# chathurawidanage/harp

Measured on AMD Instinct MI355X. Metric: sec/iteration K-means (N=1e8, d=100, K=1e4), lower is better.
Workload: dtype bf16; 1 GPU; model=kmeans-allreduce, N=100000000, d=100, K=10000, global_batch=100000000, parallelism=dp1

## Files before the change

### csrc/kmeans.hip

```cpp
#include "common.h"

#include <type_traits>

namespace {

constexpr float KM_BIG = 1.0e38f;
constexpr int KM_ONES = 4;

__device__ __forceinline__ float keyed(float v, unsigned idx) {
  return __uint_as_float((__float_as_uint(v) & ~0xFu) | idx);
}

template <int KS, int G, int WAVES_, int RG>
struct KMCfg {
  static constexpr int DP = KS * 16;
  static constexpr int CPR = KS * 2;
  static constexpr int TILE = RG * 32;
  static constexpr int WAVES = WAVES_;
  static constexpr int THREADS = WAVES_ * 64;
  static constexpr int TILE_BYTES = TILE * DP * 2;
  static constexpr int DMA_INSTR = TILE * CPR / 64;
  static constexpr int PTS = WAVES_ * G * 32;
  static_assert((TILE * CPR) % 64 == 0, "tile must be whole 1-KiB DMA pieces");
};

template <class C>
__device__ __forceinline__ void stage_dma(const __bf16* __restrict__ cm2, int tile, char* lds, int wave, int lane) {
#pragma unroll
  for (int j0 = 0; j0 < C::DMA_INSTR; j0 += C::WAVES) {
    const int j = j0 + wave;
    if (C::DMA_INSTR % C::WAVES == 0 || j < C::DMA_INSTR) {
      const int q = j * 64 + lane;
      const int row = q / C::CPR;
      int c = q - row * C::CPR - ((row >> 3) & 1);
      if (c < 0) c += C::CPR;
      const __bf16* src = cm2 + ((size_t)tile * C::TILE + row) * C::DP + c * 8;
      __builtin_amdgcn_global_load_lds((const void __attribute__((address_space(1)))*)src,
                                       (void __attribute__((address_space(3)))*)(lds + j * 1024), 16, 0, 0);
    }
  }
}

template <int KS, int G, int WAVES, int RG, int PIPE, int PRIO = 0>
__global__ __launch_bounds__(WAVES * 64) void kmeans_assign_kernel(
    const __bf16* __restrict__ X, long ldx, const __bf16* __restrict__ Cm2, long N, int ntiles, int tail_rg,
    int dcount, int* __restrict__ labels, float* __restrict__ sums, int ld_sums, float* __restrict__ obj_partial,
    float* __restrict__ mind) {
  using C = KMCfg<KS, G, WAVES, RG>;
  __shared__ __attribute__((aligned(16))) char smem[2 * C::TILE_BYTES + WAVES * 4];
  const int tid = threadIdx.x, lane = tid & 63, wave = tid >> 6;
  const int r = lane & 31, h = lane >> 5;
  const int srot = (r >> 3) & 1;
  const long pbase = ((long)blockIdx.x * WAVES + wave) * (G * 32);

  if constexpr (PRIO)
    if (__builtin_amdgcn_readfirstlane(tid) >= WAVES * 32) __builtin_amdgcn_s_setprio(1);
  stage_dma<C>(Cm2, 0, smem, wave, lane);

  bf16x8 xf[G][KS];
#pragma unroll
  for (int g = 0; g < G; ++g) {
    long p = pbase + g * 32 + r;
    if (p > N - 1) p = N - 1;
    const bf16x8* row = (const bf16x8*)(X + p * ldx);
#pragma unroll
    for (int s = 0; s < KS; ++s) xf[g][s] = row[2 * s + h];
  }

  float best[G];
  int bestt[G];
#pragma unroll
  for (int g = 0; g < G; ++g) { best[g] = KM_BIG; bestt[g] = 0; }
  auto tile_argmin = [&](const floatx16& ac, int g, int tg) {
    float m = keyed(ac[0], 0u);
#pragma unroll
    for (int q = 1; q < 16; ++q) m = fminf(m, keyed(ac[q], (unsigned)q));
    if (m < best[g]) { best[g] = m; bestt[g] = tg; }
  };

  int aoff[KS];
#pragma unroll
  for (int s = 0; s < KS; ++s) {
    int cp = 2 * s + h + srot;
    if (cp >= C::CPR) cp -= C::CPR;
    aoff[s] = (r * C::CPR + cp) * 16;
  }

  asm volatile("s_waitcnt vmcnt(0)" ::: "memory");
  __syncthreads();

  const int nfull = tail_rg ? ntiles - 1 : ntiles;
  for (int t = 0; t < nfull; ++t) {
    if (t + 1 < ntiles) stage_dma<C>(Cm2, t + 1, smem + ((t + 1) & 1) * C::TILE_BYTES, wave, lane);
    const char* buf = smem + (t & 1) * C::TILE_BYTES;
    bf16x8 af[2][KS];
#pragma unroll
    for (int s = 0; s < KS; ++s) af[0][s] = *(const bf16x8*)(buf + aoff[s]);
    if constexpr (PIPE > 0) {
      constexpr int NI = RG * G;
      floatx16 acc[2];
#pragma unroll
      for (int q = 0; q < 16; ++q) acc[0][q] = 0.f;
#pragma unroll
      for (int s = 0; s < KS; ++s) acc[0] = __builtin_amdgcn_mfma_f32_32x32x16_bf16(af[0][s], xf[0][s], acc[0], 0, 0, 0);
#pragma unroll
      for (int i = 0; i < NI; ++i) {
        const int rg = i / G, g = i % G;
        if (g == 0 && rg + 1 < RG) {
          const char* nb = buf + (rg + 1) * 32 * C::CPR * 16;
#pragma unroll
          for (int s = 0; s < KS; ++s) af[(rg + 1) & 1][s] = *(const bf16x8*)(nb + aoff[s]);
        }
        if (i + 1 < NI) {
          const int rg1 = (i + 1) / G, g1 = (i + 1) % G;
          floatx16& an = acc[(i + 1) & 1];
#pragma unroll
          for (int q = 0; q < 16; ++q) an[q] = 0.f;
#pragma unroll
          for (int s = 0; s < KS; ++s) an = __builtin_amdgcn_mfma_f32_32x32x16_bf16(af[rg1 & 1][s], xf[g1][s], an, 0, 0, 0);
        }
        tile_argmin(acc[i & 1], g, t * RG + rg);
        if constexpr (PIPE == 2) {
#pragma unroll
          for (int s = 0; s < KS; ++s) {
            __builtin_amdgcn_sched_group_barrier(0x008, 1, 0);
            __builtin_amdgcn_sched_group_barrier(0x002, 4, 0);
          }
        }
      }
    } else
#pragma unroll
    for (int rg = 0; rg < RG; ++rg) {
      if (rg + 1 < RG) {
        const char* nb = buf + (rg + 1) * 32 * C::CPR * 16;
#pragma unroll
        for (int s = 0; s < KS; ++s) af[(rg + 1) & 1][s] = *(const bf16x8*)(nb + aoff[s]);
      }
      const int tg = t * RG + rg;
#pragma unroll
      for (int g = 0; g < G; ++g) {
        floatx16 acc = {0.f, 0.f, 0.f, 0.f, 0.f, 0.f, 0.f, 0.f, 0.f, 0.f, 0.f, 0.f, 0.f, 0.f, 0.f, 0.f};
#pragma unroll
        for (int s = 0; s < KS; ++s)
          acc = __builtin_amdgcn_mfma_f32_32x32x16_bf16(af[rg & 1][s], xf[g][s], acc, 0, 0, 0);
        tile_argmin(acc, g, tg);
      }
    }
    asm volatile("s_waitcnt vmcnt(0)" ::: "memory");
    __syncthreads();
  }
  if (tail_rg) {
    const int t = ntiles - 1;
    const char* buf = smem + (t & 1) * C::TILE_BYTES;
    for (int rg = 0; rg < tail_rg; ++rg) {
      const char* nb = buf + rg * 32 * C::CPR * 16;
      bf16x8 af[KS];
#pragma unroll
      for (int s = 0; s < KS; ++s) af[s] = *(const bf16x8*)(nb + aoff[s]);
      const int tg = t * RG + rg;
#pragma unroll
      for (int g = 0; g < G; ++g) {
        floatx16 acc = {0.f, 0.f, 0.f, 0.f, 0.f, 0.f, 0.f, 0.f, 0.f, 0.f, 0.f, 0.f, 0.f, 0.f, 0.f, 0.f};
#pragma unroll
        for (int s = 0; s < KS; ++s) acc = __builtin_amdgcn_mfma_f32_32x32x16_bf16(af[s], xf[g][s], acc, 0, 0, 0);
        tile_argmin(acc, g, tg);
      }
    }
  }

  int lab[G];
  float local_obj = 0.f;
#pragma unroll
  for (int g = 0; g < G; ++g) {
    float xs = 0.f;
#pragma unroll
    for (int s = 0; s < KS; ++s)
#pragma unroll
      for (int j = 0; j < 8; ++j) {
        const float v = (float)xf[g][s][j];
        xs = fmaf(v, v, xs);
      }
    xs += __shfl_xor(xs, 32, 64);
    xs -= (float)KM_ONES;
    const float ob = __shfl_xor(best[g], 32, 64);
    const int obt = __shfl_xor(bestt[g], 32, 64);
    const bool take = h ? (ob <= best[g]) : (ob < best[g]);
    const float bv = take ? ob : best[g];
    const int bt = take ? obt : bestt[g];
    const int hw = take ? (1 - h) : h;
    const unsigned reg = __float_as_uint(bv) & 0xFu;
    const int idx = bt * 32 + (int)(reg & 3u) + 8 * (int)(reg >> 2) + 4 * hw;
    lab[g] = idx;
    const long p = pbase + g * 32 + r;
    if (h == 0 && p < N) {
      labels[p] = idx;
      local_obj += fmaxf(bv + xs, 0.f);
      if (mind) mind[p] = bv + xs;
    }
  }
  if (obj_partial) {
    local_obj = wave_sum(local_obj);
    float* red = (float*)(smem + 2 * C::TILE_BYTES);
    if (lane == 0) red[wave] = local_obj;
    __syncthreads();
    if (tid == 0) {
      float acc = 0.f;
#pragma unroll
      for (int w = 0; w < WAVES; ++w) acc += red[w];
      obj_partial[blockIdx.x] = acc;
    }
  }

  if (sums) {
#pragma unroll
    for (int g = 0; g < G; ++g) {
      for (int i = 0; i < 32; ++i) {
        const long p = pbase + g * 32 + i;
        if (p >= N) break;
        const int l = __shfl(lab[g], i, 64);
        const __bf16* xr = X + p * ldx;
        float* sr = sums + (long)l * ld_sums;
        for (int c = lane; c <= dcount; c += 64) atomicAdd(sr + c, (float)xr[c]);
      }
    }
  }
}

__global__ void kmeans_normalize_kernel(const float* __restrict__ sums, int ld, float* __restrict__ c,
                                        int Kr, int d, float* __restrict__ counts) {
  const int row = blockIdx.x * (blockDim.x >> 6) + (threadIdx.x >> 6);
  const int lane = threadIdx.x & 63;
  if (row >= Kr) return;
  const float cnt = sums[(long)row * ld + d];
  if (counts && lane == 0) counts[row] = cnt;
  if (cnt > 0.f) {
    const float inv = 1.0f / cnt;
    for (int j = lane; j < d; j += 64) c[(long)row * d + j] = sums[(long)row * ld + j] * inv;
  }
}

__global__ void kmeans_prepare_kernel(const float* __restrict__ c, int K, int d, int Kp, int dp,
                                      __bf16* __restrict__ Cm2, float* __restrict__ cn) {
  const int row = blockIdx.x * (blockDim.x >> 6) + (threadIdx.x >> 6);
  const int lane = threadIdx.x & 63;
  if (row >= Kp) return;
  float s = 0.f;
  for (int j = lane; j < d; j += 64) {
    float v = row < K ? c[(long)row * d + j] : 0.f;
    const float bf = (float)(__bf16)v;
    s = fmaf(bf, bf, s);
    Cm2[(long)row * dp + j] = (__bf16)(-2.0f * bf);
  }
  s = wave_sum(s);
  if (row >= K) s = KM_BIG;
  const __bf16 hi = (__bf16)s;
  const float r1 = s - (float)hi;
  const __bf16 mid = (__bf16)r1;
  const __bf16 lo = (__bf16)(r1 - (float)mid);
  for (int j = d + lane; j < dp; j += 64) {
    __bf16 v = (__bf16)0.f;
    if (j == d + 1) v = hi;
    else if (j == d + 2) v = mid;
    else if (j == d + 3) v = lo;
    Cm2[(long)row * dp + j] = v;
  }
  if (lane == 0) cn[row] = s;
}

__device__ __forceinline__ unsigned long long splitmix64(unsigned long long z) {
  z += 0x9E3779B97F4A7C15ull;
  z = (z ^ (z >> 30)) * 0xBF58476D1CE4E5B9ull;
  z = (z ^ (z >> 27)) * 0x94D049BB133111EBull;
  return z ^ (z >> 31);
}

__global__ void uniform_rows_bf16_kernel(__bf16* __restrict__ X, long N, int d, int dp, float lo,
                                         float hi, unsigned long long seed, long row0, int one_col) {
  const long total = N * (long)dp;
  for (long i = blockIdx.x * (long)blockDim.x + threadIdx.x; i < total; i += (long)gridDim.x * blockDim.x) {
    const long row = i / dp;
    const int col = (int)(i - row * dp);
    float v = 0.f;
    if (col < d) {
      const unsigned long long z = splitmix64(seed ^ ((unsigned long long)(row0 + row) * 0x100000001B3ull + col));
      v = lo + (hi - lo) * (float)((z >> 40) * (1.0 / 16777216.0));
    } else if (one_col && col < d + KM_ONES) {
      v = 1.0f;
    }
    X[i] = (__bf16)v;
  }
}

constexpr int KW_CB = 256, KW_RG = KW_CB / 32;

template <int G, int DC>
struct KWCfg {
  static constexpr int KS = DC / 16;
  static constexpr int CPR = DC / 8;
  static constexpr int TILE_BYTES = KW_CB * DC * 2;
  static constexpr int DMA = KW_CB * CPR / 64;
  static constexpr int PTS = 4 * G * 32;
};

template <int CPR>
__device__ __forceinline__ int wide_rot(int row) {
  return CPR == 4 ? (row >> 2) & 3 : CPR == 8 ? (row >> 1) & 7 : CPR == 16 ? row & 15 : (row >> 3) & 1;
}

template <class C>
__device__ __forceinline__ void stage_dma_wide(const __bf16* __restrict__ cm2, int dp, int row0, int kp, int f,
                                               char* lds, int wave, int lane) {
#pragma unroll
  for (int j0 = 0; j0 < C::DMA; j0 += 4) {
    const int j = j0 + wave;
    const int q = j * 64 + lane;
    const int row = q / C::CPR;
    int c = q - row * C::CPR - wide_rot<C::CPR>(row);
    if (c < 0) c += C::CPR;
    int gr = row0 + row;
    if (gr > kp - 1) gr = kp - 1;
    const __bf16* src = cm2 + (size_t)gr * dp + f * (C::CPR * 8) + c * 8;
    __builtin_amdgcn_global_load_lds((const void __attribute__((address_space(1)))*)src,
                                     (void __attribute__((address_space(3)))*)(lds + j * 1024), 16, 0, 0);
  }
}

template <int G, int DC, int OCC>
__global__ __launch_bounds__(256, OCC) void kmeans_assign_wide_kernel(
    const __bf16* __restrict__ X, long ldx, const __bf16* __restrict__ Cm2, long N, int dp, int kswept, int kp,
    int nkb, unsigned long long* __restrict__ keys) {
  using C = KWCfg<G, DC>;
  constexpr int KS = C::KS;
  __shared__ __attribute__((aligned(16))) char smem[2 * C::TILE_BYTES];
  const int tid = threadIdx.x, lane = tid & 63, wave = tid >> 6;
  const int r = lane & 31, h = lane >> 5;
  const int srot = (r >> 3) & 1;
  const long id = blockIdx.x;
  const long xcd = id & 7, round = id >> 3;
  const long pb = (round / nkb) * 8 + xcd;
  const int kb = (int)(round % nkb);
  const long npb = (N + C::PTS - 1) / C::PTS;
  if (pb >= npb) return;
  const int row0 = kb * KW_CB;
  const int live_rg = (kswept - row0) >= KW_CB ? KW_RG : (kswept - row0 + 31) / 32;
  const long pbase = pb * C::PTS + wave * (G * 32);
  const int nst = dp / DC;

  stage_dma_wide<C>(Cm2, dp, row0, kp, 0, smem, wave, lane);
  const bf16x8* xrow[G];
#pragma unroll
  for (int g = 0; g < G; ++g) {
    long p = pbase + g * 32 + r;
    if (p > N - 1) p = N - 1;
    xrow[g] = (const bf16x8*)(X + p * ldx);
  }
  bf16x8 xf[2][G][KS];
#pragma unroll
  for (int g = 0; g < G; ++g)
#pragma unroll
    for (int k = 0; k < KS; ++k) xf[0][g][k] = xrow[g][2 * k + h];
  floatx16 acc[KW_RG][G];
#pragma unroll
  for (int a = 0; a < KW_RG; ++a)
#pragma unroll
    for (int g = 0; g < G; ++g)
#pragma unroll
// ... 285 lines not shown
                                       (void __attribute__((address_space(3)))*)(xb + j * 1024), 16, 0, 0);
    }
  };
  floatx16 acc[RGW][G];
#pragma unroll
  for (int a = 0; a < RGW; ++a)
#pragma unroll
    for (int g = 0; g < G; ++g)
#pragma unroll
      for (int q = 0; q < 16; ++q) acc[a][g][q] = 0.f;
  int aoff[KS];
#pragma unroll
  for (int k = 0; k < KS; ++k) aoff[k] = (r * CPR + (2 * k + h + wide_rot<CPR>(r)) % CPR) * 16;
#pragma unroll
  for (int q = 0; q < NBUF - 1; ++q)
    if (q < nst) issue(q, q);
  float xs[G];
#pragma unroll
  for (int g = 0; g < G; ++g) xs[g] = 0.f;
  for (int f = 0; f < nst; ++f) {
    const int younger = (nst - 1 - f) < (NBUF - 2) ? (nst - 1 - f) : (NBUF - 2);
    if (younger >= 2) asm volatile("s_waitcnt vmcnt(%0)" ::"n"(2 * OPS) : "memory");
    else if (younger == 1) asm volatile("s_waitcnt vmcnt(%0)" ::"n"(OPS) : "memory");
    else asm volatile("s_waitcnt vmcnt(0)" ::: "memory");
    __syncthreads();
    if (f + NBUF - 1 < nst) issue(f + NBUF - 1, (f + NBUF - 1) % NBUF);
    const char* buf = smem + (f % NBUF) * SBYTES;
    const char* xb = buf + C::TILE_BYTES + pwo * CPR * 16;
    const char* cb = buf + rgo * 32 * CPR * 16;
    bf16x8 xf[G][KS];
#pragma unroll
    for (int g = 0; g < G; ++g)
#pragma unroll
      for (int k = 0; k < KS; ++k) xf[g][k] = *(const bf16x8*)(xb + g * 32 * CPR * 16 + aoff[k]);
#pragma unroll
    for (int g = 0; g < G; ++g)
#pragma unroll
      for (int k = 0; k < KS; ++k)
#pragma unroll
        for (int j = 0; j < 8; ++j) xs[g] = fmaf((float)xf[g][k][j], (float)xf[g][k][j], xs[g]);
    bf16x8 af[2][KS];
#pragma unroll
    for (int k = 0; k < KS; ++k) af[0][k] = *(const bf16x8*)(cb + aoff[k]);
#pragma unroll
    for (int rg = 0; rg < RGW; ++rg) {
      if (rg + 1 < RGW) {
        const char* nb = cb + (rg + 1) * 32 * CPR * 16;
#pragma unroll
        for (int k = 0; k < KS; ++k) af[(rg + 1) & 1][k] = *(const bf16x8*)(nb + aoff[k]);
      }
      if (rg < live_rg) {
#pragma unroll
        for (int g = 0; g < G; ++g)
#pragma unroll
          for (int k = 0; k < KS; ++k)
            acc[rg][g] = __builtin_amdgcn_mfma_f32_32x32x16_bf16(af[rg & 1][k], xf[g][k], acc[rg][g], 0, 0, 0);
      }
    }
  }
  float xsg[G];
#pragma unroll
  for (int g = 0; g < G; ++g) xsg[g] = xs[g] + __shfl_xor(xs[g], 32, 64) - (float)KM_ONES;
#pragma unroll
  for (int g = 0; g < G; ++g) {
    float best = KM_BIG;
    int bestt = 0;
#pragma unroll
    for (int rg = 0; rg < RGW; ++rg) {
      if (rg >= live_rg) break;
      float m = keyed(acc[rg][g][0], 0u);
#pragma unroll
      for (int q = 1; q < 16; ++q) m = fminf(m, keyed(acc[rg][g][q], (unsigned)q));
      if (m < best) {
        best = m;
        bestt = rg;
      }
    }
    const float ob = __shfl_xor(best, 32, 64);
    const int obt = __shfl_xor(bestt, 32, 64);
    const bool take = h ? (ob <= best) : (ob < best);
    const float bv = take ? ob : best;
    const int bt = take ? obt : bestt;
    const int hw = take ? (1 - h) : h;
    const unsigned reg = __float_as_uint(bv) & 0xFu;
    const int idx = row0 + (rgo + bt) * 32 + (int)(reg & 3u) + 8 * (int)(reg >> 2) + 4 * hw;
    const long p = pbase + g * 32 + r;
    if (h == 0 && p < N && live_rg > 0) {
      const float dist = fmaxf(bv + xsg[g], 0.f);
      const unsigned long long key = ((unsigned long long)__float_as_uint(dist) << 32) | (unsigned)idx;
      __hip_atomic_fetch_min(keys + p, key, __ATOMIC_RELAXED, __HIP_MEMORY_SCOPE_AGENT);
    }
  }
}

template <int G, int DC, int NBUF>
int launch_wide8(const void* X, long ldx, const void* Cm2, long N, int dp, int kswept, int kp,
                 unsigned long long* keys, hipStream_t s) {
  constexpr int XROWS = 4 * G * 32;
  if (dp % DC || (ldx * 2) % 16) return HARP_EBADARG;
  const long npb = (N + XROWS - 1) / XROWS;
  const int nkb = (kswept + KW_CB - 1) / KW_CB;
  const long rounds = (npb + 7) / 8 * nkb;
  kmeans_assign_wide8_kernel<G, DC, NBUF><<<dim3((unsigned)(rounds * 8)), dim3(512), 0, s>>>(
      (const __bf16*)X, ldx, (const __bf16*)Cm2, N, dp, kswept, kp, nkb, keys);
  return harp_launch_status();
}

template <int G, int DC, int NBUF>
int launch_wide_lds(const void* X, long ldx, const void* Cm2, long N, int dp, int kswept, int kp,
                    unsigned long long* keys, hipStream_t s) {
  constexpr int XROWS = 4 * G * 32;
  constexpr int SBYTES = KW_CB * DC * 2 + XROWS * DC * 2;
  if (dp % DC || (ldx * 2) % 16) return HARP_EBADARG;
  const long npb = (N + XROWS - 1) / XROWS;
  const int nkb = (kswept + KW_CB - 1) / KW_CB;
  const long rounds = (npb + 7) / 8 * nkb;
  (void)SBYTES;
  kmeans_assign_wide_lds_kernel<G, DC, NBUF><<<dim3((unsigned)(rounds * 8)), dim3(256), 0, s>>>(
      (const __bf16*)X, ldx, (const __bf16*)Cm2, N, dp, kswept, kp, nkb, keys);
  return harp_launch_status();
}

template <int G, int DC, int OCC>
int launch_wide(const void* X, long ldx, const void* Cm2, long N, int dp, int kswept, int kp,
                unsigned long long* keys, hipStream_t s) {
  using C = KWCfg<G, DC>;
  if (dp % DC) return HARP_EBADARG;
  const long npb = (N + C::PTS - 1) / C::PTS;
  const int nkb = (kswept + KW_CB - 1) / KW_CB;
  const long rounds = (npb + 7) / 8 * nkb;
  kmeans_assign_wide_kernel<G, DC, OCC><<<dim3((unsigned)(rounds * 8)), dim3(256), 0, s>>>(
      (const __bf16*)X, ldx, (const __bf16*)Cm2, N, dp, kswept, kp, nkb, keys);
  return harp_launch_status();
}

__global__ __launch_bounds__(256) void kmeans_wide_finish_kernel(const unsigned long long* __restrict__ keys, long N,
                                                                 int* __restrict__ labels, float* __restrict__ obj_partial,
                                                                 float* __restrict__ mind) {
  __shared__ float red[4];
  const long p = blockIdx.x * 256L + threadIdx.x;
  float v = 0.f;
  if (p < N) {
    const unsigned long long k = keys[p];
    labels[p] = (int)(k & 0xffffffffull);
    v = __uint_as_float((unsigned)(k >> 32));
    if (mind) mind[p] = v;
  }
  v = wave_sum(v);
  if ((threadIdx.x & 63) == 0) red[threadIdx.x >> 6] = v;
  __syncthreads();
  if (threadIdx.x == 0 && obj_partial) obj_partial[blockIdx.x] = red[0] + red[1] + red[2] + red[3];
}

template <int KS, int G, int WAVES, int RG, int PIPE = 0, int PRIO = 0>
int launch_assign(const void* X, long ldx, const void* Cm2, long N, int Kp, int d, int* labels, float* sums,
                  int ld_sums, float* obj_partial, float* mind, hipStream_t stream) {
  using C = KMCfg<KS, G, WAVES, RG>;
  if (Kp % 32) return HARP_EBADARG;
  const long nblk = (N + C::PTS - 1) / C::PTS;
  const int ntiles = (Kp + C::TILE - 1) / C::TILE, tail_rg = (Kp % C::TILE) / 32;
  kmeans_assign_kernel<KS, G, WAVES, RG, PIPE, PRIO><<<dim3((unsigned)nblk), dim3(C::THREADS), 0, stream>>>(
      (const __bf16*)X, ldx, (const __bf16*)Cm2, N, ntiles, tail_rg, d, labels, sums, ld_sums, obj_partial, mind);
  return harp_launch_status();
}

#define KM_VARIANTS(KS)                                                                       \
  switch (variant) {                                                                        \
    case 4: return launch_assign<KS, 1, 16, 2>(X, ldx, Cm2, N, Kp, d, labels, sums, ld, op, md, s);  \
    case 13: return launch_assign<KS, 4, 8, 2, 2>(X, ldx, Cm2, N, Kp, d, labels, sums, ld, op, md, s); \
    case 14: return launch_assign<KS, 4, 8, 4, 2>(X, ldx, Cm2, N, Kp, d, labels, sums, ld, op, md, s); \
    case 15: return launch_assign<KS, 4, 8, 4, 2, 1>(X, ldx, Cm2, N, Kp, d, labels, sums, ld, op, md, s); \
    default: return HARP_EBADARG;                                                           \
  }

}

HARP_EXPORT int harp_kmeans_points_per_block(int variant) {
  switch (variant) {
    case 4: return 16 * 1 * 32;
    case 13: case 14: case 15: return 8 * 4 * 32;
    default: return -1;
  }
}

HARP_EXPORT int harp_kmeans_assign(const void* X, long ldx, const void* Cm2, long N, int dp, int Kp, int d,
                                   int* labels, float* sums, int ld, float* op, float* md, int variant,
                                   hipStream_t s) {
  if (N <= 0 || d + KM_ONES > dp || dp % 16 || Kp <= 0 || Kp % 32 || ldx < dp || ldx % 8) return HARP_EBADARG;
  switch (dp / 16) {
    case 1: KM_VARIANTS(1)
    case 2: KM_VARIANTS(2)
    case 3: KM_VARIANTS(3)
    case 4: KM_VARIANTS(4)
    case 5: KM_VARIANTS(5)
    case 6: KM_VARIANTS(6)
    case 7: KM_VARIANTS(7)
    case 8: KM_VARIANTS(8)
#define KM_WIDE(KSV) case KSV: return launch_assign<KSV, 1, 16, 2>(X, ldx, Cm2, N, Kp, d, labels, sums, ld, op, md, s);
    KM_WIDE(9) KM_WIDE(10) KM_WIDE(11) KM_WIDE(12) KM_WIDE(13) KM_WIDE(14) KM_WIDE(15) KM_WIDE(16)
#undef KM_WIDE
    default: return HARP_EUNSUPPORTED;
  }
}

HARP_EXPORT int harp_kmeans_assign_wide(const void* X, long ldx, const void* Cm2, long N, int dp, int kswept, int kp,
                                        int d, unsigned long long* keys, int variant, hipStream_t s) {
  if (N <= 0 || d + KM_ONES > dp || dp % 64 || dp <= 0 || kswept <= 0 || kswept % 32 || kp < kswept ||
      ldx < dp || ldx % 8 || !keys)
    return HARP_EBADARG;
  if (variant == 0) variant = 6;
  switch (variant) {
    case 1: return launch_wide<2, 64, 1>(X, ldx, Cm2, N, dp, kswept, kp, keys, s);
    case 3: return launch_wide<1, 64, 2>(X, ldx, Cm2, N, dp, kswept, kp, keys, s);
    case 5: return launch_wide_lds<2, 64, 2>(X, ldx, Cm2, N, dp, kswept, kp, keys, s);
    case 6: return launch_wide8<2, 64, 2>(X, ldx, Cm2, N, dp, kswept, kp, keys, s);
    default: return HARP_EBADARG;
  }
}

HARP_EXPORT int harp_kmeans_wide_finish(const unsigned long long* keys, long N, int* labels, float* obj_partial,
                                        float* mind, hipStream_t s) {
  if (N <= 0) return HARP_OK;
  kmeans_wide_finish_kernel<<<dim3((unsigned)((N + 255) / 256)), dim3(256), 0, s>>>(keys, N, labels, obj_partial, mind);
  return harp_launch_status();
}

HARP_EXPORT int harp_kmeans_normalize(const float* sums, int ld, float* c, int Kr, int d, float* counts,
                                      hipStream_t s) {
  if (Kr <= 0) return HARP_OK;
  const int wpb = 4;
  kmeans_normalize_kernel<<<dim3((Kr + wpb - 1) / wpb), dim3(64 * wpb), 0, s>>>(sums, ld, c, Kr, d, counts);
  return harp_launch_status();
}

HARP_EXPORT int harp_kmeans_prepare(const float* c, int K, int d, int Kp, int dp, void* Cm2, float* cn,
                                    hipStream_t s) {
  if (Kp < K || dp < d) return HARP_EBADARG;
  const int wpb = 4;
  kmeans_prepare_kernel<<<dim3((Kp + wpb - 1) / wpb), dim3(64 * wpb), 0, s>>>(c, K, d, Kp, dp, (__bf16*)Cm2, cn);
  return harp_launch_status();
}

HARP_EXPORT int harp_uniform_rows_bf16(void* X, long N, int d, int dp, float lo, float hi,
                                       unsigned long long seed, long row0, int one_col, hipStream_t s) {
  if (N <= 0) return HARP_OK;
  long blocks = (N * (long)dp + 255) / 256;
  if (blocks > 65536) blocks = 65536;
  uniform_rows_bf16_kernel<<<dim3((unsigned)blocks), dim3(256), 0, s>>>((__bf16*)X, N, d, dp, lo, hi, seed, row0,
                                                                       one_col);
  return harp_launch_status();
}
```

### harp_amd/ops/kmeans.py

```python
from __future__ import annotations

import math
import os
from dataclasses import dataclass
from typing import Optional

import torch

from . import _lib

KP_ALIGN = 128
ONES = 4
DEFAULT_VARIANT = 15


NARROW_MAX_DP = 256
WIDE_ALIGN = 64
WIDE_VARIANT = int(os.environ.get("HARP_KMEANS_WIDE_VARIANT", "0"))


def padded_dim(d: int) -> int:
    dp = (d + ONES + 15) // 16 * 16
    return dp if dp <= NARROW_MAX_DP else (d + ONES + WIDE_ALIGN - 1) // WIDE_ALIGN * WIDE_ALIGN


def padded_k(k: int) -> int:
    return (k + KP_ALIGN - 1) // KP_ALIGN * KP_ALIGN


def row_stride(dp: int) -> int:
    return (dp + 127) // 128 * 128


def pack_points(x: torch.Tensor, device: torch.device | str | None = None) -> torch.Tensor:
    device = torch.device(device) if device is not None else x.device
    n, d = x.shape
    dp = padded_dim(d)
    dt = torch.bfloat16 if device.type == "cuda" else torch.float32
    ld = row_stride(dp) if device.type == "cuda" else dp
    out = torch.zeros((n, ld), dtype=dt, device=device)
    out[:, :d] = x.to(device=device, dtype=dt)
    out[:, d:d + ONES] = 1.0
    return out[:, :dp]


def generate_points(n: int, d: int, lo: float = 0.0, hi: float = 1000.0, seed: int = 0,
                    device: torch.device | str = "cpu", row0: int = 0) -> torch.Tensor:
    device = torch.device(device)
    dp = padded_dim(d)
    if device.type == "cuda" and _lib.use_native(torch.empty(0, device=device)):
        ld = row_stride(dp)
        Xs = torch.empty((n, ld), dtype=torch.bfloat16, device=device)
        _lib.check(_lib.kernels().harp_uniform_rows_bf16(Xs.data_ptr(), n, d, ld, float(lo), float(hi),
                                                         seed & 0xFFFFFFFFFFFFFFFF, row0, 1,
                                                         _lib.stream_ptr(device)), "uniform_rows")
        return Xs[:, :dp]
    g = torch.Generator().manual_seed(seed * 1000003 + row0)
    x = torch.rand((n, d), generator=g, dtype=torch.float32) * (hi - lo) + lo
    return pack_points(x, device)


_SIDE: dict = {}


def pipeline_chunks(n: int, ppb: int) -> int:
    c = int(os.environ.get("HARP_KMEANS_CHUNKS", "1"))
    return max(1, min(c, n // (ppb * 256)))


def _side_stream(dev: torch.device) -> torch.cuda.Stream:
    s = _SIDE.get(dev)
    if s is None:
        s = _SIDE[dev] = torch.cuda.Stream(dev)
    return s


@dataclass
class CentroidOperand:
    Cm2: torch.Tensor
    cn: torch.Tensor
    K: int
    d: int


def prepare(c: torch.Tensor, dp: int, out: Optional[CentroidOperand] = None) -> CentroidOperand:
    K, d = c.shape
    Kp = padded_k(K)
    dev = c.device
    if out is None:
        dt = torch.bfloat16 if dev.type == "cuda" else torch.float32
        out = CentroidOperand(torch.empty((Kp, dp), dtype=dt, device=dev), torch.empty(Kp, dtype=torch.float32, device=dev), K, d)
    if _lib.use_native(c):
        cc = c.contiguous().float()
        _lib.check(_lib.kernels().harp_kmeans_prepare(cc.data_ptr(), K, d, Kp, dp, out.Cm2.data_ptr(),
                                                      out.cn.data_ptr(), _lib.stream_ptr(dev)), "kmeans_prepare")
        return out
    out.Cm2.zero_()
    out.Cm2[:K, :d] = -2.0 * c
    out.cn.fill_(1e38)
    out.cn[:K] = (c.double() ** 2).sum(1).float()
    return out


def swept_k(op: "CentroidOperand") -> int:
    return min(op.Cm2.shape[0], (op.K + 31) // 32 * 32)


def _assign_wide(X, op, sums, labels, want_objective, obj_partial, min_dist):
    n, dp = X.shape
    dev = X.device
    lib = _lib.kernels()
    assert X.dtype == torch.bfloat16 and X.stride(1) == 1 and X.stride(0) % 8 == 0 and op.Cm2.shape[1] == dp
    assert dp % WIDE_ALIGN == 0, f"wide rows need dp % {WIDE_ALIGN} == 0 (pack with padded_dim)"
    keys = torch.full((n,), -1, dtype=torch.int64, device=dev)
    _lib.check(lib.harp_kmeans_assign_wide(X.data_ptr(), X.stride(0), op.Cm2.data_ptr(), n, dp, swept_k(op),
                                           op.Cm2.shape[0], op.d, keys.data_ptr(), WIDE_VARIANT, _lib.stream_ptr(dev)),
               "kmeans_assign_wide")
    nblk = (n + 255) // 256
    if want_objective and (obj_partial is None or obj_partial.numel() < nblk):
        obj_partial = torch.empty(nblk, dtype=torch.float32, device=dev)
    _lib.check(lib.harp_kmeans_wide_finish(keys.data_ptr(), n, labels.data_ptr(),
                                           obj_partial.data_ptr() if want_objective else None,
                                           min_dist.data_ptr() if min_dist is not None else None,
                                           _lib.stream_ptr(dev)), "kmeans_wide_finish")
    if sums is not None:
        from . import segment

        assert sums.dtype == torch.float32 and sums.shape[1] >= op.d + 1 and sums.is_contiguous()
        assert sums.shape[0] >= op.Cm2.shape[0], "sums needs Kp (padded) rows"
        assert sums.device == dev
        perm, start = segment.bucket_labels(labels, op.Cm2.shape[0])
        segment.bucket_rowsum(X, perm, start, sums)
    obj = obj_partial[:nblk].double().sum() if want_objective else None
    return labels, obj


def assign(X: torch.Tensor, op: CentroidOperand, sums: Optional[torch.Tensor] = None,
           labels: Optional[torch.Tensor] = None, want_objective: bool = True, variant: int = DEFAULT_VARIANT,
           obj_partial: Optional[torch.Tensor] = None, accumulate: str = "bucket",
           min_dist: Optional[torch.Tensor] = None):
    n, dp = X.shape
    dev = X.device
    if labels is None:
        labels = torch.empty(n, dtype=torch.int32, device=dev)
    if _lib.use_native(X):
        lib = _lib.kernels()
        if dp > NARROW_MAX_DP:
            if accumulate == "atomic":
                raise ValueError("accumulate='atomic' is only fused into the narrow kernel (dp <= "
                                 f"{NARROW_MAX_DP}); the wide path (dp = {dp}) accumulates by bucket")
            return _assign_wide(X, op, sums, labels, want_objective, obj_partial, min_dist)
        if dp > 128:
            variant = 4
        elif variant in (14, 15) and dp // 16 == 5:
            variant = 13
        ppb = lib.harp_kmeans_points_per_block(variant)
        if ppb <= 0:
            raise ValueError(f"unknown kmeans kernel variant {variant}")
        nblk = (n + ppb - 1) // ppb
        if want_objective and (obj_partial is None or obj_partial.numel() < nblk):
            obj_partial = torch.empty(nblk, dtype=torch.float32, device=dev)
        if sums is not None:
            assert sums.dtype == torch.float32 and sums.shape[1] >= op.d + 1 and sums.is_contiguous()
            assert sums.shape[0] >= op.Cm2.shape[0], "sums needs Kp (padded) rows"
            assert sums.device == dev
        assert X.dtype == torch.bfloat16 and X.stride(1) == 1 and X.stride(0) % 8 == 0 and op.Cm2.shape[1] == dp
        fused = sums if accumulate == "atomic" else None
        bucket = sums is not None and fused is None
        chunks = pipeline_chunks(n, ppb) if bucket else 1
        per = max(1, (nblk + chunks - 1) // chunks) * ppb
        side = _side_stream(dev) if chunks > 1 else None
        main = torch.cuda.current_stream(dev)
        for r0 in range(0, n, per):
            r1 = min(n, r0 + per)
            b0 = r0 // ppb
            st = lib.harp_kmeans_assign(X[r0].data_ptr(), X.stride(0), op.Cm2.data_ptr(), r1 - r0, dp,
                                        swept_k(op), op.d,
                                        labels[r0].data_ptr(), _lib.ptr(fused),
                                        fused.stride(0) if fused is not None else 0,
                                        obj_partial[b0].data_ptr() if want_objective else None,
                                        min_dist[r0].data_ptr() if min_dist is not None else None, variant,
                                        _lib.stream_ptr(dev))
            _lib.check(st, "kmeans_assign")
            if not bucket:
                continue
            from . import segment

            if side is None:
                perm, start = segment.bucket_labels(labels, op.Cm2.shape[0])
                segment.bucket_rowsum(X, perm, start, sums)
                continue
            side.wait_stream(main)
            with torch.cuda.stream(side):
                perm, start = segment.bucket_labels(labels[r0:r1], op.Cm2.shape[0])
                segment.bucket_rowsum(X[r0:r1], perm, start, sums)
        if side is not None:
            main.wait_stream(side)
        obj = obj_partial[:nblk].double().sum() if want_objective else None
        return labels, obj
    Xf = X.float()
    d = op.d
    x = Xf[:, :d]
    C = -0.5 * op.Cm2[: op.K, :d].float()
    dist = op.cn[: op.K].unsqueeze(0) - 2.0 * (x @ C.t())
    lab = dist.argmin(1)
    labels.copy_(lab.to(labels.dtype))
    if min_dist is not None:
        min_dist.copy_((dist.gather(1, lab[:, None])[:, 0] + (x * x).sum(1)).to(min_dist.dtype))
    if sums is not None:
        sums[:, : d + 1].index_add_(0, lab, Xf[:, : d + 1])
    obj = None
    if want_objective:
        xs = (x.double() ** 2).sum(1)
        obj = (dist.gather(1, lab[:, None])[:, 0].double() + xs).clamp_min(0).sum()
    return labels, obj


def normalize(sums: torch.Tensor, c: torch.Tensor, d: int, counts: Optional[torch.Tensor] = None) -> torch.Tensor:
    Kr = c.shape[0]
    if _lib.use_native(c):
        assert sums.is_contiguous() and c.is_contiguous()
        _lib.check(_lib.kernels().harp_kmeans_normalize(sums.data_ptr(), sums.stride(0), c.data_ptr(), Kr, d,
                                                        _lib.ptr(counts), _lib.stream_ptr(c.device)),
                   "kmeans_normalize")
        return c
    cnt = sums[:, d]
    m = cnt > 0
    c[m] = sums[m, :d] / cnt[m, None]
    if counts is not None:
        counts.copy_(cnt)
    return c
```

### harp_amd/ops/segment.py

```python
from __future__ import annotations

import ctypes
import os
from typing import Dict, Tuple

import torch

from . import _lib

_lib.register({
    "harp_bucket_chunk": [_lib.c_long],
    "harp_bucket_workspace_ints": [_lib.c_long, _lib.c_int],
    "harp_bucket_labels": [_lib.c_void_p, _lib.c_long, _lib.c_int, _lib.c_void_p, _lib.c_void_p, _lib.c_void_p,
                           _lib.c_void_p],
    "harp_bucket_rowsum_bf16": [_lib.c_void_p, _lib.c_int, _lib.c_long, _lib.c_void_p, _lib.c_void_p, _lib.c_int,
                                _lib.c_long, _lib.c_void_p, _lib.c_int, _lib.c_void_p],
})
_WS: Dict[Tuple, torch.Tensor] = {}


def _lib_ret_long(fn):
    fn.restype = ctypes.c_long
    return fn


def bucket_labels(labels: torch.Tensor, K: int) -> Tuple[torch.Tensor, torch.Tensor]:
    n = labels.numel()
    if not _lib.use_native(labels):
        order = torch.argsort(labels.long(), stable=True)
        counts = torch.bincount(labels.long(), minlength=K)
        start = torch.zeros(K + 1, dtype=torch.int64)
        start[1:] = torch.cumsum(counts, 0)
        return order.to(torch.int32), start.to(torch.int32)
    lib = _lib.kernels()
    _lib_ret_long(lib.harp_bucket_workspace_ints)
    need = lib.harp_bucket_workspace_ints(n, K)
    stream = torch.cuda.current_stream(labels.device).cuda_stream
    key = (labels.device, n, K, stream)
    ws = _WS.get(key)
    if ws is None:
        for k in [k for k in _WS if k[3] == stream]:
            del _WS[k]
        ws = torch.empty(need, dtype=torch.int32, device=labels.device)
        _WS[key] = ws
    so, po = ctypes.c_long(0), ctypes.c_long(0)
    st = lib.harp_bucket_labels(labels.data_ptr(), n, K, ws.data_ptr(), ctypes.byref(so), ctypes.byref(po),
                                _lib.stream_ptr(labels.device))
    _lib.check(st, "bucket_labels")
    return ws[po.value:po.value + n], ws[so.value:so.value + K + 1]


SUM_SLICE = min(1024, max(8, int(os.environ.get("HARP_ROWSUM_SLICE", "1024")) // 8 * 8))


def bucket_rowsum(X: torch.Tensor, perm: torch.Tensor, start: torch.Tensor, out: torch.Tensor) -> torch.Tensor:
    K = start.numel() - 1
    if not _lib.use_native(X):
        idx = torch.repeat_interleave(torch.arange(K), (start[1:] - start[:-1]).long())
        out[:K, : X.shape[1]].index_add_(0, idx, X[perm.long()].float())
        return out
    assert X.dtype == torch.bfloat16 and X.stride(1) == 1 and out.dtype == torch.float32 and out.is_contiguous()
    for c0 in range(0, X.shape[1], SUM_SLICE):
        w = min(SUM_SLICE, X.shape[1] - c0)
        st = _lib.kernels().harp_bucket_rowsum_bf16(X[:, c0:].data_ptr(), w, X.stride(0), perm.data_ptr(),
                                                    start.data_ptr(), K, perm.numel(), out[:, c0:].data_ptr(),
                                                    out.stride(0), _lib.stream_ptr(X.device))
        _lib.check(st, "bucket_rowsum")
    return out
```

Baseline: 0.1443 s/iter.

## Add keyless assign variant with group-level argmin and fused resolve-rowsum kernel

The assign kernel gets a keyless mode that takes a plain fminf over each 32-centroid tile and keeps only the tile index, instead of packing the row index into the low mantissa bits. Labels become group ids, points are bucketed by group, and a new kernel recomputes the exact row within each 32-centroid group with a small MFMA. The same kernel accumulates centroid sums through a one-hot MFMA and flushes them with atomics. This is meant to cut the per-element keying work in the hot argmin loop, at the cost of a second distance pass per point, extra bucketing over fewer groups, and chunked processing of N.

```diff
diff --git a/csrc/kmeans.hip b/csrc/kmeans.hip
--- a/csrc/kmeans.hip
+++ b/csrc/kmeans.hip
@@ -41,7 +41,7 @@
   }
 }
 
-template <int KS, int G, int WAVES, int RG, int PIPE, int PRIO = 0>
+template <int KS, int G, int WAVES, int RG, int PIPE, int PRIO = 0, int KEYLESS = 0>
 __global__ __launch_bounds__(WAVES * 64) void kmeans_assign_kernel(
     const __bf16* __restrict__ X, long ldx, const __bf16* __restrict__ Cm2, long N, int ntiles, int tail_rg,
     int dcount, int* __restrict__ labels, float* __restrict__ sums, int ld_sums, float* __restrict__ obj_partial,
@@ -72,9 +72,16 @@
 #pragma unroll
   for (int g = 0; g < G; ++g) { best[g] = KM_BIG; bestt[g] = 0; }
   auto tile_argmin = [&](const floatx16& ac, int g, int tg) {
-    float m = keyed(ac[0], 0u);
-#pragma unroll
-    for (int q = 1; q < 16; ++q) m = fminf(m, keyed(ac[q], (unsigned)q));
+    float m;
+    if constexpr (KEYLESS) {
+      m = ac[0];
+#pragma unroll
+      for (int q = 1; q < 16; ++q) m = fminf(m, ac[q]);
+    } else {
+      m = keyed(ac[0], 0u);
+#pragma unroll
+      for (int q = 1; q < 16; ++q) m = fminf(m, keyed(ac[q], (unsigned)q));
+    }
     if (m < best[g]) { best[g] = m; bestt[g] = tg; }
   };
 
@@ -184,12 +191,13 @@
     xs -= (float)KM_ONES;
     const float ob = __shfl_xor(best[g], 32, 64);
     const int obt = __shfl_xor(bestt[g], 32, 64);
-    const bool take = h ? (ob <= best[g]) : (ob < best[g]);
+    const bool take = KEYLESS ? (ob < best[g] || (ob == best[g] && obt < bestt[g]))
+                              : (h ? (ob <= best[g]) : (ob < best[g]));
     const float bv = take ? ob : best[g];
     const int bt = take ? obt : bestt[g];
     const int hw = take ? (1 - h) : h;
     const unsigned reg = __float_as_uint(bv) & 0xFu;
-    const int idx = bt * 32 + (int)(reg & 3u) + 8 * (int)(reg >> 2) + 4 * hw;
+    const int idx = KEYLESS ? bt : bt * 32 + (int)(reg & 3u) + 8 * (int)(reg >> 2) + 4 * hw;
     lab[g] = idx;
     const long p = pbase + g * 32 + r;
     if (h == 0 && p < N) {
@@ -211,7 +219,7 @@
     }
   }
 
-  if (sums) {
+  if (!KEYLESS && sums) {
 #pragma unroll
     for (int g = 0; g < G; ++g) {
       for (int i = 0; i < 32; ++i) {
@@ -803,14 +811,14 @@
   if (threadIdx.x == 0 && obj_partial) obj_partial[blockIdx.x] = red[0] + red[1] + red[2] + red[3];
 }
 
-template <int KS, int G, int WAVES, int RG, int PIPE = 0, int PRIO = 0>
+template <int KS, int G, int WAVES, int RG, int PIPE = 0, int PRIO = 0, int KEYLESS = 0>
 int launch_assign(const void* X, long ldx, const void* Cm2, long N, int Kp, int d, int* labels, float* sums,
                   int ld_sums, float* obj_partial, float* mind, hipStream_t stream) {
   using C = KMCfg<KS, G, WAVES, RG>;
-  if (Kp % 32) return HARP_EBADARG;
+  if (Kp % 32 || (KEYLESS && sums)) return HARP_EBADARG;
   const long nblk = (N + C::PTS - 1) / C::PTS;
   const int ntiles = (Kp + C::TILE - 1) / C::TILE, tail_rg = (Kp % C::TILE) / 32;
-  kmeans_assign_kernel<KS, G, WAVES, RG, PIPE, PRIO><<<dim3((unsigned)nblk), dim3(C::THREADS), 0, stream>>>(
+  kmeans_assign_kernel<KS, G, WAVES, RG, PIPE, PRIO, KEYLESS><<<dim3((unsigned)nblk), dim3(C::THREADS), 0, stream>>>(
       (const __bf16*)X, ldx, (const __bf16*)Cm2, N, ntiles, tail_rg, d, labels, sums, ld_sums, obj_partial, mind);
   return harp_launch_status();
 }
@@ -821,6 +829,7 @@
     case 13: return launch_assign<KS, 4, 8, 2, 2>(X, ldx, Cm2, N, Kp, d, labels, sums, ld, op, md, s); \
     case 14: return launch_assign<KS, 4, 8, 4, 2>(X, ldx, Cm2, N, Kp, d, labels, sums, ld, op, md, s); \
     case 15: return launch_assign<KS, 4, 8, 4, 2, 1>(X, ldx, Cm2, N, Kp, d, labels, sums, ld, op, md, s); \
+    case 16: return launch_assign<KS, 4, 8, 4, 2, 1, 1>(X, ldx, Cm2, N, Kp, d, labels, sums, ld, op, md, s); \
     default: return HARP_EBADARG;                                                           \
   }
 
@@ -829,7 +838,7 @@
 HARP_EXPORT int harp_kmeans_points_per_block(int variant) {
   switch (variant) {
     case 4: return 16 * 1 * 32;
-    case 13: case 14: case 15: return 8 * 4 * 32;
+    case 13: case 14: case 15: case 16: return 8 * 4 * 32;
     default: return -1;
   }
 }
diff --git a/csrc/kmeans_resolve.hip b/csrc/kmeans_resolve.hip
--- /dev/null
+++ b/csrc/kmeans_resolve.hip
@@ -0,0 +1,168 @@
+#include "common.h"
+
+namespace {
+
+constexpr int KR_RUN = 2048;
+
+template <int KS>
+__global__ __launch_bounds__(64) __attribute__((amdgpu_waves_per_eu(3))) void kmeans_resolve_rowsum_kernel(
+    const __bf16* __restrict__ X, long ldx, const __bf16* __restrict__ Cm2, const int* __restrict__ perm,
+    const int* __restrict__ start, int NG, long n, int* __restrict__ labels, float* __restrict__ sums, int ld) {
+  constexpr int DP = KS * 16;
+  constexpr int NCB = (DP + 31) / 32;
+  constexpr int STRE = NCB * 32 + 8;
+  __shared__ __attribute__((aligned(16))) __bf16 tile[32 * STRE];
+  __shared__ bf16x8 atile[KS * 64];
+  const int lane = threadIdx.x;
+  const int c = lane & 31, h = lane >> 5;
+  const long j0 = (long)blockIdx.x * KR_RUN;
+  if (j0 >= n) return;
+  const long j1 = j0 + KR_RUN < n ? j0 + KR_RUN : n;
+
+  for (int i = lane; i < 32 * STRE; i += 64) tile[i] = (__bf16)0.f;
+  int lo = 0, hi = NG;
+  while (hi - lo > 1) {
+    const int mid = (lo + hi) >> 1;
+    if (start[mid] <= j0) lo = mid; else hi = mid;
+  }
+  int k = lo;
+  long kend = start[k + 1];
+  int kloaded = -1;
+  bool dirty = false;
+  floatx16 S[NCB];
+#pragma unroll
+  for (int b = 0; b < NCB; ++b)
+#pragma unroll
+    for (int q = 0; q < 16; ++q) S[b][q] = 0.f;
+
+  auto pos = [&](long jb) {
+    const long j = jb + c;
+    return j < j1 ? j : j1 - 1;
+  };
+  auto load_rows = [&](bf16x8 (&xf)[KS], int p) {
+    const bf16x8* row = (const bf16x8*)(X + (long)p * ldx);
+#pragma unroll
+    for (int s = 0; s < KS; ++s) xf[s] = row[2 * s + h];
+  };
+  auto flush = [&](int kk) {
+    float* o = sums + ((long)kk * 32 + 4 * h) * ld + c;
+#pragma unroll
+    for (int b = 0; b < NCB; ++b) {
+#pragma unroll
+      for (int q = 0; q < 16; ++q) {
+        const int rq = (q & 3) + 8 * (q >> 2);
+        if (32 * b + c < DP && S[b][q] != 0.f) atomicAdd(o + (long)rq * ld + 32 * b, S[b][q]);
+        S[b][q] = 0.f;
+      }
+    }
+  };
+
+  bf16x8 xp[KS];
+  int pp = perm[pos(j0)];
+  int pn = perm[pos(j0 + 32)];
+  load_rows(xp, pp);
+
+  for (long jb = j0; jb < j1; jb += 32) {
+    const long je = jb + 32 < j1 ? jb + 32 : j1;
+    const long jj = jb + c;
+    __syncthreads();
+#pragma unroll
+    for (int s = 0; s < KS; ++s) *(bf16x8*)(tile + c * STRE + (2 * s + h) * 8) = xp[s];
+    const int pc = pp;
+    if (jb + 32 < j1) load_rows(xp, pn);
+    pp = pn;
+    pn = perm[pos(jb + 64)];
+    __syncthreads();
+    long cur = jb;
+    while (cur < je) {
+      while (cur >= kend) {
+        if (dirty) {
+          flush(k);
+          dirty = false;
+        }
+        ++k;
+        kend = start[k + 1];
+      }
+      if (k != kloaded) {
+        const bf16x8* arow = (const bf16x8*)(Cm2 + ((long)k * 32 + c) * DP);
+#pragma unroll
+        for (int s = 0; s < KS; ++s) atile[s * 64 + lane] = arow[2 * s + h];
+        kloaded = k;
+      }
+      const long sub_end = kend < je ? kend : je;
+      const bool mine = jj >= cur && jj < sub_end;
+      floatx16 acc = {0.f, 0.f, 0.f, 0.f, 0.f, 0.f, 0.f, 0.f, 0.f, 0.f, 0.f, 0.f, 0.f, 0.f, 0.f, 0.f};
+#pragma unroll
+      for (int s = 0; s < KS; ++s) {
+        acc = __builtin_amdgcn_mfma_f32_32x32x16_bf16(atile[s * 64 + lane],
+                                                      *(const bf16x8*)(tile + c * STRE + (2 * s + h) * 8), acc, 0, 0, 0);
+        __builtin_amdgcn_sched_barrier(0);
+      }
+      float m = acc[0];
+      int mq = 0;
+#pragma unroll
+      for (int q = 1; q < 16; ++q)
+        if (acc[q] < m) {
+          m = acc[q];
+          mq = q;
+        }
+      int row = (mq & 3) + 8 * (mq >> 2) + 4 * h;
+      const float om = __shfl_xor(m, 32, 64);
+      const int orow = __shfl_xor(row, 32, 64);
+      if (om < m || (om == m && orow < row)) row = orow;
+      if (mine && h == 0) labels[pc] = k * 32 + row;
+      const int code = mine ? row : -1;
+#pragma unroll
+      for (int t = 0; t < 2; ++t) {
+        bf16x8 oh;
+#pragma unroll
+        for (int j = 0; j < 8; ++j) {
+          const int r0 = __builtin_amdgcn_readlane(code, 16 * t + j), r1 = __builtin_amdgcn_readlane(code, 16 * t + 8 + j);
+          oh[j] = (__bf16)((h ? r1 : r0) == c ? 1.f : 0.f);
+        }
+        const __bf16* tp = tile + (16 * t + 8 * h) * STRE + c;
+#pragma unroll
+        for (int b = 0; b < NCB; ++b) {
+          bf16x8 xt;
+#pragma unroll
+          for (int j = 0; j < 8; ++j) xt[j] = tp[j * STRE + 32 * b];
+          S[b] = __builtin_amdgcn_mfma_f32_32x32x16_bf16(oh, xt, S[b], 0, 0, 0);
+          __builtin_amdgcn_sched_barrier(0);
+        }
+      }
+      dirty = true;
+      cur = sub_end;
+    }
+  }
+  if (dirty) flush(k);
+}
+
+template <int KS>
+int launch_resolve(const void* X, long ldx, const void* Cm2, const int* perm, const int* start, int NG, long n,
+                   int* labels, float* sums, int ld, hipStream_t s) {
+  const long nblk = (n + KR_RUN - 1) / KR_RUN;
+  kmeans_resolve_rowsum_kernel<KS><<<dim3((unsigned)nblk), dim3(64), 0, s>>>(
+      (const __bf16*)X, ldx, (const __bf16*)Cm2, perm, start, NG, n, labels, sums, ld);
+  return harp_launch_status();
+}
+
+}
+
+HARP_EXPORT int harp_kmeans_resolve_rowsum(const void* X, long ldx, const void* Cm2, int dp, const int* perm,
+                                           const int* start, int NG, long n, int* labels, float* sums, int ld,
+                                           hipStream_t s) {
+  if (n <= 0) return n == 0 ? HARP_OK : HARP_EBADARG;
+  if (dp <= 0 || dp % 16 || dp > 128 || ldx < dp || ldx % 8 || ld < dp || NG <= 0 || !labels || !sums)
+    return HARP_EBADARG;
+  switch (dp / 16) {
+    case 1: return launch_resolve<1>(X, ldx, Cm2, perm, start, NG, n, labels, sums, ld, s);
+    case 2: return launch_resolve<2>(X, ldx, Cm2, perm, start, NG, n, labels, sums, ld, s);
+    case 3: return launch_resolve<3>(X, ldx, Cm2, perm, start, NG, n, labels, sums, ld, s);
+    case 4: return launch_resolve<4>(X, ldx, Cm2, perm, start, NG, n, labels, sums, ld, s);
+    case 5: return launch_resolve<5>(X, ldx, Cm2, perm, start, NG, n, labels, sums, ld, s);
+    case 6: return launch_resolve<6>(X, ldx, Cm2, perm, start, NG, n, labels, sums, ld, s);
+    case 7: return launch_resolve<7>(X, ldx, Cm2, perm, start, NG, n, labels, sums, ld, s);
+    case 8: return launch_resolve<8>(X, ldx, Cm2, perm, start, NG, n, labels, sums, ld, s);
+    default: return HARP_EUNSUPPORTED;
+  }
+}
diff --git a/harp_amd/ops/kmeans.py b/harp_amd/ops/kmeans.py
--- a/harp_amd/ops/kmeans.py
+++ b/harp_amd/ops/kmeans.py
@@ -11,7 +11,10 @@
 
 KP_ALIGN = 128
 ONES = 4
-DEFAULT_VARIANT = 15
+DEFAULT_VARIANT = 16
+KEYLESS_VARIANT, KEYED_VARIANT = 16, 15
+KEYLESS_MAX_DP = 128
+RESOLVE_SPAN = 1 << 23
 
 
 NARROW_MAX_DP = 256
@@ -150,6 +153,10 @@
                 raise ValueError("accumulate='atomic' is only fused into the narrow kernel (dp <= "
                                  f"{NARROW_MAX_DP}); the wide path (dp = {dp}) accumulates by bucket")
             return _assign_wide(X, op, sums, labels, want_objective, obj_partial, min_dist)
+        keyless = (variant == KEYLESS_VARIANT and dp <= KEYLESS_MAX_DP and sums is not None
+                   and accumulate == "bucket" and min_dist is None)
+        if variant == KEYLESS_VARIANT and not keyless:
+            variant = KEYED_VARIANT
         if dp > 128:
             variant = 4
         elif variant in (14, 15) and dp // 16 == 5:
@@ -186,14 +193,22 @@
                 continue
             from . import segment
 
+            def bucket_sum(lab, Xc):
+                if keyless:
+                    for s0 in range(0, lab.numel(), RESOLVE_SPAN):
+                        ls, Xs = lab[s0:s0 + RESOLVE_SPAN], Xc[s0:s0 + RESOLVE_SPAN]
+                        perm, start = segment.bucket_labels(ls, swept_k(op) // 32)
+                        segment.resolve_rowsum(Xs, op.Cm2, perm, start, ls, sums)
+                else:
+                    perm, start = segment.bucket_labels(lab, op.Cm2.shape[0])
+                    segment.bucket_rowsum(Xc, perm, start, sums)
+
             if side is None:
-                perm, start = segment.bucket_labels(labels, op.Cm2.shape[0])
-                segment.bucket_rowsum(X, perm, start, sums)
+                bucket_sum(labels, X)
                 continue
             side.wait_stream(main)
             with torch.cuda.stream(side):
-                perm, start = segment.bucket_labels(labels[r0:r1], op.Cm2.shape[0])
-                segment.bucket_rowsum(X[r0:r1], perm, start, sums)
+                bucket_sum(labels[r0:r1], X[r0:r1])
         if side is not None:
             main.wait_stream(side)
         obj = obj_partial[:nblk].double().sum() if want_objective else None
diff --git a/harp_amd/ops/segment.py b/harp_amd/ops/segment.py
--- a/harp_amd/ops/segment.py
+++ b/harp_amd/ops/segment.py
@@ -15,6 +15,9 @@
                            _lib.c_void_p],
     "harp_bucket_rowsum_bf16": [_lib.c_void_p, _lib.c_int, _lib.c_long, _lib.c_void_p, _lib.c_void_p, _lib.c_int,
                                 _lib.c_long, _lib.c_void_p, _lib.c_int, _lib.c_void_p],
+    "harp_kmeans_resolve_rowsum": [_lib.c_void_p, _lib.c_long, _lib.c_void_p, _lib.c_int, _lib.c_void_p,
+                                   _lib.c_void_p, _lib.c_int, _lib.c_long, _lib.c_void_p, _lib.c_void_p, _lib.c_int,
+                                   _lib.c_void_p],
 })
 _WS: Dict[Tuple, torch.Tensor] = {}
 
@@ -38,6 +41,9 @@
     stream = torch.cuda.current_stream(labels.device).cuda_stream
     key = (labels.device, n, K, stream)
     ws = _WS.get(key)
+    if ws is None:
+        ws = next((w for k, w in _WS.items() if k[0] == labels.device and k[3] == stream and w.numel() >= need),
+                  None)
     if ws is None:
         for k in [k for k in _WS if k[3] == stream]:
             del _WS[k]
@@ -67,3 +73,18 @@
                                                     out.stride(0), _lib.stream_ptr(X.device))
         _lib.check(st, "bucket_rowsum")
     return out
+
+
+def resolve_rowsum(X: torch.Tensor, Cm2: torch.Tensor, perm: torch.Tensor, start: torch.Tensor,
+                   labels: torch.Tensor, out: torch.Tensor) -> torch.Tensor:
+    NG = start.numel() - 1
+    dp = X.shape[1]
+    assert X.dtype == torch.bfloat16 and X.stride(1) == 1 and out.dtype == torch.float32 and out.is_contiguous()
+    assert Cm2.dtype == torch.bfloat16 and Cm2.is_contiguous() and Cm2.shape[1] == dp and Cm2.shape[0] >= 32 * NG
+    assert out.shape[0] >= 32 * NG and labels.dtype == torch.int32 and labels.is_contiguous()
+    assert labels.numel() == perm.numel() == X.shape[0]
+    st = _lib.kernels().harp_kmeans_resolve_rowsum(X.data_ptr(), X.stride(0), Cm2.data_ptr(), dp, perm.data_ptr(),
+                                                   start.data_ptr(), NG, perm.numel(), labels.data_ptr(),
+                                                   out.data_ptr(), out.stride(0), _lib.stream_ptr(X.device))
+    _lib.check(st, "kmeans_resolve_rowsum")
+    return out
```

Result: faster. 0.1382 s/iter, median of 6 (-4.2%).
